# metagentools/VStrains

Measured on AMD Instinct MI355X. Metric: PE read pairs/sec through PE-link inference (GFA index + packed reads in HBM -> node_mat/short_mat), higher is better.
Workload: dtype u32

## Files before the change

vstrains_amd/csrc/vs_pe.hip:

```cpp
#include <stdio.h>
#include <stdlib.h>
#include <string.h>

#include <vector>

#include "vs_internal.h"
#include "vs_acc_tasks.h"
#include "vs_pe_pack.h"

#define TPB 256
#define LCAP 20u
__device__ __forceinline__ const uint32_t *vs_row_quad(const uint32_t *__restrict__ lists, const uint32_t *__restrict__ hi, uint64_t row, uint32_t q) {
    return q < LC / 4u ? lists + row * LC + 4u * q : hi + row * 4u;
}
#define EMPTY_NODE 0xFFFFFFFFu

struct PeParams {
    VsIndexDev idx;
    VsReadsDev rd;
    uint32_t *node_mat, *short_mat;
    unsigned long long *stats;
    uint32_t ept, pmax, words_cap, pool, pool_bits;
    uint64_t n_tiles;
    uint32_t *slow_list, *slow_count;
// ... 531 lines not shown
            __syncthreads();
            if (it < NI) {
                s_pcnt[it] = cnt;
                s_pa[it] = pa;
                s_pb[it] = pb;
            }
        } else
        for (uint32_t it = ltop; it < NI; it += TTPB) {
            uint32_t e = STD ? it / STD_PMAX : vs_fastdiv(it, P.magic_pmax), pi = it - e * pmax;
            uint32_t cnt = 0, pa = 0, pb = 0;
            const uint32_t est = e < ne ? s_state[e] : 0u;
            if ((est & 3u) == 1u) {
                uint32_t meta = s_meta[e];
                uint32_t rlen = meta & VS_LEN_MASK;
                uint32_t j = (est >> 8) + pi * s;
                if (j + w <= rlen) {
                    uint32_t sr;
                    const uint64_t key = vs_seed_key(s_words, e * wpe * 16u + j, w, &sr);
                    bool ok = true;
                    if ((meta >> 24) & VS_FLAG_INVALID) {
                        if (FAST) {
                            uint32_t lo, hi;
                            ok = vs_seed_limits(s_inv[e], j, w, rlen, &lo, &hi);
                        } else {
                            ok = !vs_seed_dirty(P.rd.mask, (uint64_t)s_gwoff[e] * 16u + j, w);
                        }
                    }
                    if (ok) cnt = vs_probe(P.idx, key, sr, &pa, &pb);
                }
            }
            s_pcnt[it] = cnt;
            s_pa[it] = pa;
            s_pb[it] = pb;
        }
        __syncthreads();
        {
            const uint32_t chunk = (NI + TTPB - 1u) / TTPB;
            const uint32_t b = ltop * chunk;
            uint32_t local = 0;
            for (uint32_t i = 0; i < chunk; i++)
                if (b + i < NI) local += s_pcnt[b + i];
            const uint32_t incl = vs_wave_scan_add(local);
            const uint32_t lane = ltop & 63u;
            if (lane == 63u) s_misc[ltop >> 6] = incl;
            __syncthreads();
            uint32_t off = incl - local;
            for (uint32_t wv = 0; wv < (ltop >> 6); wv++) off += s_misc[wv];
            for (uint32_t i = 0; i < chunk; i++)
                if (b + i < NI) {
                    off += s_pcnt[b + i];
                    s_pcnt[b + i] = off;
                }
        }
        __syncthreads();
        {
        const uint32_t total = s_pcnt[NI - 1u];
        for (uint32_t c0 = 0; c0 < total; c0 += KCHUNK) {
            for (uint32_t i = tid; i < KCHUNK; i += TTPB) s_owner[i] = 0;
            __syncthreads();
            for (uint32_t it = tid; it < NI; it += TTPB) {
                const uint32_t incl = s_pcnt[it], excl = s_pcnt[(int)it - 1];
                if (incl > excl) {
                    const uint32_t lo = excl > c0 ? excl : c0;
                    const uint32_t hi = incl < c0 + KCHUNK ? incl : c0 + KCHUNK;
                    if (lo < hi) s_owner[lo - c0] = it + 1u;
                }
            }
            __syncthreads();
            uint32_t own[KPPT];
            uint32_t run = 0;
#pragma unroll
            for (uint32_t k2 = 0; k2 < KPPT; k2++) {
                const uint32_t v = s_owner[tid * KPPT + k2];
                run = v > run ? v : run;
                own[k2] = run;
            }
            const uint32_t incl = vs_wave_scan_max(run);
            const uint32_t lane = tid & 63u;
            if (lane == 63u) s_misc[4u + (tid >> 6)] = incl;
            uint32_t carry = __shfl_up(incl, 1, 64);
            if (lane == 0u) carry = 0;
            __syncthreads();
            {
                const uint32_t wv = tid >> 6;
#pragma unroll
                for (uint32_t pw = 0; pw + 1u < TTPB / 64u; pw++) {
                    const uint32_t mw = s_misc[4u + pw];
                    if (wv > pw) carry = mw > carry ? mw : carry;
                }
            }
            bool live[KPPT];
            uint32_t p_e[KPPT], p_j[KPPT], p_node[KPPT], p_pos[KPPT], p_opp[KPPT];
            VsNodeMeta p_nm[KPPT];
#pragma unroll
            for (uint32_t k2 = 0; k2 < KPPT; k2++) {
                const uint32_t t = c0 + tid * KPPT + k2;
                live[k2] = t < total;
                const uint32_t it = live[k2] ? (own[k2] > carry ? own[k2] : carry) - 1u : 0u;
                const uint32_t excl = s_pcnt[(int)it - 1];
                const uint32_t cnt = s_pcnt[it] - excl;
                const uint32_t pa = s_pa[it], pb = s_pb[it];
                const uint32_t e = STD ? it / STD_PMAX : vs_fastdiv(it, P.magic_pmax), pi = it - e * pmax;
                p_e[k2] = e;
                uint32_t gap = s;
                {
                    const uint32_t est = s_state[e];
                    if (ADAPT) {
                        const uint32_t D = est >> 20, t = (est >> 16) & 15u;
                        p_j[k2] = ((est >> 8) & 0xFFu) + pi * s - (pi >= t ? D : 0u);
                        if (pi && pi == t) gap = s - D;
                    } else {
                        p_j[k2] = (est >> 8) + pi * s;
                    }
                }
                uint32_t node = pa, pos = pb & 0x7FFFFFFFu, opp = pb >> 31;
                p_nm[k2].woff = 0; p_nm[k2].len = 0;
                if (live[k2] && cnt != 1u) {
                    const VsPosting po = vs_posting_unpack(P.idx.postings[pa + (t - excl)]);
                    node = po.node; pos = po.pos; opp = po.strand ^ (pb >> 31);
                    p_nm[k2].woff = po.woff; p_nm[k2].len = po.len;
                } else if (live[k2]) {
                    if (P.shortcut && s <= w && pi) {
                        const uint32_t excl2 = s_pcnt[(int)it - 2];
                        if (excl - excl2 == 1u && s_pa[it - 1u] == node) {
                            const uint32_t pbp = s_pb[it - 1u];
                            const uint32_t want = opp ? pos + gap : pos - gap;
                            if ((pbp >> 31) == opp && (pbp & 0x7FFFFFFFu) == want && (opp || pos >= gap)) live[k2] = false;
                        }
                    }
                    if (live[k2]) p_nm[k2] = P.idx.meta[node];
                }
                p_node[k2] = node; p_pos[k2] = pos; p_opp[k2] = opp;
                if (ADAPT) p_j[k2] |= gap << 16;
            }
#pragma unroll
            for (uint32_t k2 = 0; k2 < KPPT; k2++) {
                if (!live[k2]) continue;
                const uint32_t e = p_e[k2], j = ADAPT ? p_j[k2] & 0xFFFFu : p_j[k2], node = p_node[k2], opp = p_opp[k2];
                const uint32_t gap = ADAPT ? p_j[k2] >> 16 : s;
                VsNodeMeta nm = p_nm[k2];
                const uint32_t meta = s_meta[e];
                const uint32_t rlen = meta & VS_LEN_MASK;
                const uint32_t *tw = P.idx.fwd_words;
                const uint32_t q = opp ? nm.len - p_pos[k2] - w : p_pos[k2];
                uint32_t a, qa, len;
                if (FAST) {
                    uint32_t lo = 0u, hi = rlen;
                    if ((meta >> 24) & VS_FLAG_INVALID) vs_seed_limits(s_inv[e], j, w, rlen, &lo, &hi);
                    uint32_t cl = gap < j - lo ? gap : j - lo;
                    cl = cl < q ? cl : q;
                    uint32_t rem = hi - j - wv;
                    const uint32_t dr = nm.len - q - wv;
                    rem = rem < dr ? rem : dr;
                    uint32_t left = 0u, ext = 0u;
                    const uint32_t tb = (nm.woff + (opp ? P.idx.rc_delta : 0u)) * 16u;
                    if (MODE == 2) vs_agree_long(s_words, e * wpe * 16u, tw, tb + q, cl, tb + q + wv, rem, j, wv, &left, &ext);
                    else vs_agree_fast<STD>(s_words, e * wpe * 16u, tw, tb + q, cl, tb + q + wv, rem, j, wv, &left, &ext);
                    len = left + wv + ext;
                    if (left >= gap || len < K) continue;
                    a = j - left;
                    qa = q - left;
                } else {
                    const uint32_t tb = (nm.woff + (opp ? P.idx.rc_delta : 0u)) * 16u;
                    const uint32_t *mk = ((meta >> 24) & VS_FLAG_INVALID) ? P.rd.mask : nullptr;
                    if (!vs_extend(s_words, e * wpe * 16u, rlen, tw, tb, nm.len, j, q, wv, s, K, mk, (uint64_t)s_gwoff[e] * 16u, &a, &qa, &len))
                        continue;
                }
                credit(e, node, nm.len, len - K + 1u, opp ? nm.len - qa - len : qa, a);
            }
            __syncthreads();
        }
        }
        __builtin_amdgcn_s_waitcnt(0x0F70);
        __syncthreads();
        uint32_t lt = tid;
        asm volatile("" : "+v"(lt));
        constexpr uint32_t SPT = STD ? C_POOL / TTPB : 1u;
        uint32_t r_key[SPT], r_at[SPT];
        auto judge = [&](uint32_t i, uint32_t key) -> uint32_t {
            const uint32_t e = key >> 25, node = key & 0x01FFFFFFu;
            const uint32_t rlen = s_meta[e] & VS_LEN_MASK;
            const uint32_t hj = s_hminj[i];
            const uint32_t nlen = FAST ? hj >> AB : P.idx.meta[node].len;
            const uint32_t minj = FAST ? hj & ((1u << AB) - 1u) : hj;
            if (FAST ? vs_accept32(s_hcnt[i], s_hminp[i], minj, nlen, rlen, K) : vs_accept(s_hcnt[i], s_hminp[i], minj, nlen, rlen, K))
                return atomicAdd(&s_ns[e], 1u);
            return 0xFFFFFFFFu;
        };
        if (STD) {
#pragma unroll
            for (uint32_t j = 0; j < SPT; j++) {
                const uint32_t i = lt + j * TTPB;
                r_key[j] = s_hkey[i];
                r_at[j] = r_key[j] != EMPTY_NODE ? judge(i, r_key[j]) : 0xFFFFFFFFu;
            }
        } else {
            for (uint32_t i = lt; i < pool; i += TTPB) {
                const uint32_t key = s_hkey[i];
                if (key != EMPTY_NODE) s_hcnt[i] = judge(i, key);
            }
        }
        __syncthreads();
        if (lt < 64u) {
            const uint32_t e0 = 2u * lt, e1 = e0 + 1u;
            const uint32_t st0 = e0 < ne ? s_state[e0] : 0u, st1 = e1 < ne ? s_state[e1] : 0u;
            const uint32_t n0 = (st0 & 3u) == 1u ? s_ns[e0] : 0u, n1 = (st1 & 3u) == 1u ? s_ns[e1] : 0u;
            bool over0 = n0 > LCAP, over1 = n1 > LCAP;
            const uint32_t q0 = over0 ? 0u : (n0 + 3u) >> 2, q1 = over1 ? 0u : (n1 + 3u) >> 2;
            const uint32_t incl = vs_wave_scan_add(q0 + q1);
            const uint32_t capq = (ept * LC - C_TRIM) >> 2;
            const uint32_t o0 = incl - q0 - q1, o1 = o0 + q0;
            over0 |= o0 + q0 > capq;
            over1 |= o1 + q1 > capq;
            if (e0 < ne) { s_pcnt[e0] = over0 || (st0 & 3u) != 1u ? 0xFFFFFFFFu : 4u * o0; if (over0) s_state[e0] = st0 | 2u; }
            if (e1 < ne) { s_pcnt[e1] = over1 || (st1 & 3u) != 1u ? 0xFFFFFFFFu : 4u * o1; if (over1) s_state[e1] = st1 | 2u; }
            if (lt == 63u) s_misc[8] = 4u * (incl < capq ? incl : capq);
        }
        __syncthreads();
        uint32_t *s_off = s_pcnt;
        if (STD) {
#pragma unroll
            for (uint32_t j = 0; j < SPT; j++)
                if (r_at[j] != 0xFFFFFFFFu) {
                    const uint32_t o = s_off[r_key[j] >> 25];
                    if (o != 0xFFFFFFFFu) s_list[o + r_at[j]] = r_key[j] & 0x01FFFFFFu;
                }
        } else {
            for (uint32_t i = lt; i < pool; i += TTPB) {
                const uint32_t key = s_hkey[i];
                if (key != EMPTY_NODE) {
                    const uint32_t at = s_hcnt[i], o = s_off[key >> 25];
                    if (at != 0xFFFFFFFFu && o != 0xFFFFFFFFu) s_list[o + at] = key & 0x01FFFFFFu;
                }
            }
        }
        __syncthreads();
        if (lt < npair) {
            uint32_t st = s_state[2 * lt] | s_state[2 * lt + 1];
            if ((st & 1u) && (st & 2u)) {
                uint32_t at = atomicAdd(P.slow_count, 1u);
                P.slow_list[at] = s_gend[2 * lt] >> 1;
                s_state[2 * lt] |= 2u;
                s_state[2 * lt + 1] |= 2u;
            }
        }
        __syncthreads();
        if (accumulate) {
            if (!P.out_rows) {
                uint32_t *ol = P.out_lists + (uint64_t)tile * ept * LC;
                const uint32_t total = s_misc[8];
                for (uint32_t i = lt; i < total; i += TTPB) ol[i] = s_list[i];
                for (uint32_t i = lt; i < ne; i += TTPB) {
                    const uint32_t n = (s_state[i] & 3u) == 1u ? s_ns[i] : 0u;
                    P.out_counts[(uint64_t)tile * ept + i] = n ? n | (s_off[i] >> 2) << 8 : 0u;
                }
            } else {
                uint32_t *ol = P.out_lists + (uint64_t)tile * ept * LC, *oh = P.out_lists_hi + (uint64_t)tile * ept * 4u;
                for (uint32_t i = lt; i < ne * (LCAP / 4u); i += TTPB) {
                    const uint32_t e = i / (LCAP / 4u), q4 = 4u * (i - e * (LCAP / 4u));
                    const uint32_t n = (s_state[e] & 3u) == 1u ? s_ns[e] : 0u;
                    if (q4 < n) {
                        const uint32_t *src = s_list + s_off[e] + q4;
                        *(VsQuad *)(q4 < LC ? ol + e * LC + q4 : oh + e * 4u) = VsQuad{src[0], src[1], src[2], src[3]};
                    }
                }
                for (uint32_t i = lt; i < ne; i += TTPB)
                    P.out_counts[(uint64_t)tile * ept + i] = (s_state[i] & 3u) == 1u ? s_ns[i] : 0u;
            }
        }
        if (want_dbg) {
            for (uint32_t i = tid; i < ne; i += TTPB) {
                if (s_state[i] & 2u) continue;
                uint32_t n = s_ns[i];
                const uint64_t ge = s_gend[i];
                P.dbg_counts[ge] = n;
                for (uint32_t k2 = 0; k2 < n && k2 < P.dbg_cap; k2++) P.dbg_lists[ge * P.dbg_cap + k2] = s_list[s_off[i] + k2];
            }
        }
    }
    __syncthreads();
    if (tid < 3 && P.stats && s_misc[12 + tid]) atomicAdd(&P.stats[tid], (unsigned long long)s_misc[12 + tid]);
}

#define ACC_LDS_BYTES ((2u * ACC_SLOTS + (ACC_TPB / 64) * (ACC_TASK_WORDS + ACC_BINS) + 4u) * 4u)
static_assert(ACC_LDS_BYTES <= 160u * 1024u, "k_pe_accumulate: one workgroup per CU");
template <uint32_t BITS>
struct CellTable {
    static constexpr uint32_t EMPTY = 0xFFFFFFFFu;
    __device__ static uint32_t key(uint32_t mat, uint32_t x, uint32_t y, uint32_t N) { return (mat * N + x) * N + y; }
    __device__ static uint32_t slot(uint32_t k) { return ((((k >> 4) * 0x9E3779B1u) >> (36u - BITS)) << 4) | (k & 15u); }
    __device__ static uint32_t next(uint32_t at) { return (at + 16u) & ((1u << BITS) - 1u); }
};
typedef CellTable<ACC_BITS> Acc32;

template <typename TB>
__device__ __forceinline__ bool vs_cell_claim(uint32_t *s_key, uint32_t *s_cnt, uint32_t *s_used, uint32_t key, uint32_t at, uint32_t wgt) {
    for (uint32_t pr = 0; pr < 8u; pr++) {
        uint32_t kx = s_key[at];
        if (kx == TB::EMPTY) {
            kx = atomicCAS(&s_key[at], TB::EMPTY, key);
            if (kx == TB::EMPTY) { atomicAdd(s_used, 1u); kx = key; }
        }
        if (kx == key) {
            atomicAdd(&s_cnt[at], wgt);
            return true;
        }
        at = TB::next(at);
    }
    return false;
}

template <typename TB>
__device__ __forceinline__ bool vs_cell_claim_seen(uint32_t *s_key, uint32_t *s_cnt, uint32_t *s_used, uint32_t key, uint32_t at, uint32_t wgt, uint32_t seen) {
    uint32_t kx = seen;
    for (uint32_t pr = 0; pr < 8u; pr++) {
        if (pr) kx = s_key[at];
        if (kx == TB::EMPTY) {
            kx = atomicCAS(&s_key[at], TB::EMPTY, key);
            if (kx == TB::EMPTY) { atomicAdd(s_used, 1u); kx = key; }
        }
        if (kx == key) {
            atomicAdd(&s_cnt[at], wgt);
            return true;
        }
        at = TB::next(at);
    }
    return false;
}

__device__ __forceinline__ void vs_wave_lds_sync() {
    __builtin_amdgcn_fence(__ATOMIC_RELEASE, "workgroup");
    __builtin_amdgcn_wave_barrier();
    __builtin_amdgcn_fence(__ATOMIC_ACQUIRE, "workgroup");
}

__global__ void __launch_bounds__(ACC_TPB)
k_pe_accumulate(const uint32_t *__restrict__ lists, const uint32_t *__restrict__ counts, uint64_t n_slots_pairs,
                uint32_t pairs_per_wg, uint32_t N, uint32_t use_table, uint32_t fill_limit, uint32_t task_cap,
                uint32_t *__restrict__ node_mat, uint32_t *__restrict__ short_mat, uint32_t *__restrict__ queue, uint32_t ept) {
    const uint32_t tid = threadIdx.x, lane = tid & 63u, wv = tid >> 6;
    uint32_t *s_key = vs_lds;
    uint32_t *s_cnt = vs_lds + ACC_SLOTS;
    uint32_t *s_bin = vs_lds + 2u * ACC_SLOTS + wv * (ACC_TASK_WORDS + ACC_BINS);
    uint16_t *s_task = (uint16_t *)(s_bin + ACC_BINS);
    uint32_t *s_misc = vs_lds + 2u * ACC_SLOTS + (ACC_TPB / 64) * (ACC_TASK_WORDS + ACC_BINS);
    uint32_t &s_used = s_misc[0], &s_lost = s_misc[1], &s_chunk = s_misc[2];
    const uint32_t NN = N * N;
    for (uint32_t i = tid; i < ACC_SLOTS; i += ACC_TPB) { s_key[i] = Acc32::EMPTY; s_cnt[i] = 0; }
    if (tid == 0) { s_used = 0; s_lost = 0; }
    __syncthreads();
    const uint32_t ppt = ept >> 1, region_q = (ept * LC) >> 2;
    auto write_out = [&]() {
        for (uint32_t i = tid; i < ACC_SLOTS; i += ACC_TPB) {
            const uint32_t key = s_key[i];
            if (key != Acc32::EMPTY) {
                atomicAdd(key >= NN ? short_mat + (key - NN) : node_mat + key, s_cnt[i]);
                s_key[i] = Acc32::EMPTY;
                s_cnt[i] = 0;
            }
        }
        if (tid == 0) { s_used = 0; s_lost = 0; }
        __syncthreads();
    };
    for (;;) {
    __syncthreads();
    if (tid == 0) s_chunk = atomicAdd(queue, 1u);
    __syncthreads();
    const uint64_t chunk = s_chunk;
    const uint64_t lo = chunk * pairs_per_wg;
    if (lo >= n_slots_pairs) break;
    const uint64_t hi = lo + pairs_per_wg < n_slots_pairs ? lo + pairs_per_wg : n_slots_pairs;
    for (uint64_t base = lo; base < hi; base += (ACC_TPB / 64u) * ACC_PPW) {
        const uint64_t wbase = base + wv * ACC_PPW;
        const uint32_t *wcounts = counts + 2u * wbase;
        const uint64_t tile0 = wbase / ppt;
        const uint32_t rem0 = (uint32_t)(wbase - tile0 * ppt);
        const uint32_t *wlists = lists + tile0 * ept * LC;
        uint32_t nl = 0, nr = 0, packed = 0;
        if (wbase + lane < hi) {
            const uint2 c = *(const uint2 *)(wcounts + 2u * lane);
            nl = c.x & 0xFFu; nr = c.y & 0xFFu;
            const uint32_t tq = (rem0 + lane) / ppt * region_q;
            packed = nl | nr << 5 | (tq + (c.x >> 8)) << 10 | (tq + (c.y >> 8)) << 21;
        }
        const uint32_t my_tasks = vs_acc_pair_tasks(nl, nr);
        for (uint32_t first = 0; first < ACC_PPW;) {
            const uint32_t incl = vs_wave_scan_add(lane >= first ? my_tasks : 0u);
            const uint32_t last = (uint32_t)__popcll(__ballot(vs_acc_batch_fits(incl, task_cap)));
            const uint32_t U = (uint32_t)__builtin_amdgcn_readlane((int)incl, (int)last - 1);
            const bool mine = lane >= first && lane < last;
            first = last;
            if (!U) continue;
            if (lane < ACC_BINS) s_bin[lane] = 0u;
            vs_wave_lds_sync();
            uint32_t o_n = 0, o_lm = 0, o_rm = 0, o_l[4], o_r[4];
            if (mine) {
                if (nl && nr) o_n = atomicAdd(&s_bin[nr], nl);
                if (nl & 1u) o_lm = atomicAdd(&s_bin[(nl + 1u) >> 1], 1u);
                if (nr & 1u) o_rm = atomicAdd(&s_bin[(nr + 1u) >> 1], 1u);
#pragma unroll
                for (uint32_t r = 0; r < 4u; r++) {
                    const VsAccClass cl = vs_acc_fold_class(nl, r), cr = vs_acc_fold_class(nr, r);
                    o_l[r] = cl.cnt ? atomicAdd(&s_bin[cl.turns], cl.cnt) : 0u;
                    o_r[r] = cr.cnt ? atomicAdd(&s_bin[cr.turns], cr.cnt) : 0u;
                }
            }
            vs_wave_lds_sync();
            {
                const uint32_t v = lane < ACC_BINS ? s_bin[ACC_BINS - 1u - lane] : 0u;
                const uint32_t before = vs_wave_scan_add(v) - v;
                if (lane < ACC_BINS) s_bin[ACC_BINS - 1u - lane] = before;
            }
            vs_wave_lds_sync();
            if (mine) {
                if (nl && nr) {
                    const uint32_t at = s_bin[nr] + o_n;
                    for (uint32_t a = 0; a < nl; a++) s_task[at + a] = vs_acc_task_entry(lane, VS_ACC_NODE, a);
                }
                if (nl & 1u) s_task[s_bin[(nl + 1u) >> 1] + o_lm] = vs_acc_task_entry(lane, VS_ACC_LEFT, nl >> 1);
                if (nr & 1u) s_task[s_bin[(nr + 1u) >> 1] + o_rm] = vs_acc_task_entry(lane, VS_ACC_RIGHT, nr >> 1);
                uint32_t nl2 = nl, nr2 = nr;
                asm volatile("" : "+v"(nl2), "+v"(nr2));
#pragma unroll
                for (uint32_t r = 0; r < 4u; r++) {
                    const VsAccClass cl = vs_acc_fold_class(nl2, r), cr = vs_acc_fold_class(nr2, r);
                    if (cl.cnt) {
                        const uint32_t at = s_bin[cl.turns] + o_l[r];
                        for (uint32_t i = 0; i < cl.cnt; i++) s_task[at + i] = vs_acc_task_entry(lane, VS_ACC_LEFT, cl.a0 + 4u * i);
                    }
                    if (cr.cnt) {
                        const uint32_t at = s_bin[cr.turns] + o_r[r];
                        for (uint32_t i = 0; i < cr.cnt; i++) s_task[at + i] = vs_acc_task_entry(lane, VS_ACC_RIGHT, cr.a0 + 4u * i);
                    }
                }
            }
            vs_wave_lds_sync();
            struct Task {
                uint32_t x, mat, off, p, p2, e, turns;
                VsQuad q;
            };
            auto decode = [&](uint32_t t0) {
                Task T;
                const uint32_t w = t0 + lane < U ? s_task[t0 + lane] : 0u;
                const uint32_t kind = vs_acc_entry_kind(w), a = vs_acc_entry_a(w);
                const uint32_t pk = __shfl(packed, (int)vs_acc_entry_pair(w), 64);
                const uint32_t ql = pk & 31u, qr = (pk >> 5) & 31u, rowl = ((pk >> 10) & 0x7FFu) << 2, rowr = (pk >> 21) << 2;
                const VsAccSegs s = w ? vs_acc_task_segs(kind, a, ql, qr) : VsAccSegs{0u, 0u, 0u};
                T.turns = vs_acc_turns(s);
                T.mat = kind != VS_ACC_NODE ? 1u : 0u;
                T.off = !w ? 0u : kind == VS_ACC_LEFT ? rowl : rowr;
                T.p = s.p1; T.p2 = s.p2; T.e = s.e;
                T.x = 0u;
                if (w && kind == VS_ACC_NODE) T.x = wlists[rowl + a];
                T.q = *(const VsQuad *)(wlists + T.off + T.p);
                return T;
            };
            Task nxt = decode(0u);
            for (uint32_t t0 = 0; t0 < U; t0 += 64u) {
                const Task c = nxt;
                if (t0 + 64u < U) nxt = decode(t0 + 64u);
                const uint32_t tmax = (uint32_t)__builtin_amdgcn_readlane((int)vs_wave_scan_max(c.turns), 63);
                const uint32_t mat = c.mat, e = c.e;
                const uint32_t *plist = wlists + c.off;
                uint32_t x = c.x, p = c.p, p2 = c.p2;
                bool fresh = true;
                VsQuad q = c.q;
                for (uint32_t t = 0; t < tmax; t += 4u) {
                    const uint32_t ys[4] = {q.x, q.y, q.z, q.w};
                    if (mat && fresh) x = ys[0];
                    const uint32_t pb = p;
                    p += 4u;
                    fresh = p >= e;
                    if (fresh) { p = p2; p2 = e; }
                    if (t + 4u < tmax) q = *(const VsQuad *)(plist + p);
                    const uint32_t left = tmax - t;
                    if (use_table) {
                        uint32_t key[4], seen[4], at[4];
#pragma unroll
                        for (uint32_t j = 0; j < 4u; j++) {
                            if (j >= left) break;
                            const uint32_t yv = ys[j];
                            const uint32_t cx = (mat && yv < x) ? yv : x, cy = (mat && yv < x) ? x : yv;
                            key[j] = Acc32::key(mat, cx, cy, N);
                            at[j] = Acc32::slot(key[j]);
                            seen[j] = s_key[at[j]];
                        }
#pragma unroll
                        for (uint32_t j = 0; j < 4u; j++) {
                            if (j >= left) break;
                            if (pb + j >= e) continue;
                            if (seen[j] == key[j]) {
                                atomicAdd(&s_cnt[at[j]], 1u);
                            } else if (!vs_cell_claim_seen<Acc32>(s_key, s_cnt, &s_used, key[j], at[j], 1u, seen[j])) {
                                atomicAdd(&s_lost, 1u);
                                atomicAdd(key[j] >= NN ? short_mat + (key[j] - NN) : node_mat + key[j], 1u);
                            }
                        }
                    } else {
#pragma unroll
                        for (uint32_t j = 0; j < 4u; j++) {
                            if (pb + j >= e) continue;
                            const uint32_t yv = ys[j];
                            const uint32_t cx = (mat && yv < x) ? yv : x, cy = (mat && yv < x) ? x : yv;
                            atomicAdd((mat ? short_mat : node_mat) + (uint64_t)cx * N + cy, 1u);
                        }
                    }
                }
            }
        }
        __syncthreads();
        const bool spill = s_used > fill_limit || s_lost > 4096u;
        __syncthreads();
        if (spill) write_out();
    }
    }
    __syncthreads();
    write_out();
}

__global__ void __launch_bounds__(256) k_mark_tiles(const uint32_t *__restrict__ lists, const uint32_t *__restrict__ counts,
                                                   uint64_t n_slots_pairs, uint8_t *__restrict__ map, uint32_t T, uint32_t ept) {
    const uint64_t p = (uint64_t)blockIdx.x * blockDim.x + threadIdx.x;
    if (p >= n_slots_pairs) return;
    const uint32_t cl = counts[2u * p], cr = counts[2u * p + 1u], nl = cl & 0xFFu, nr = cr & 0xFFu;
    if (!nl && !nr) return;
    const uint32_t *region = lists + 2u * p / ept * ept * LC, *rl = region + 4u * (cl >> 8), *rr = region + 4u * (cr >> 8);
    uint8_t *smap = map + (uint64_t)T * T;
    uint32_t tl[8], tr[8], kl = 0, kr = 0;
    bool over = false;
    auto put = [&](uint32_t (&tt)[8], uint32_t &k, uint32_t t) {
        bool seen = false;
#pragma unroll
        for (uint32_t j = 0; j < 8u; j++) seen |= j < k && tt[j] == t;
        if (seen) return;
        if (k >= 8u) { over = true; return; }
#pragma unroll
        for (uint32_t j = 0; j < 8u; j++)
            if (j == k) tt[j] = t;
        k++;
    };
#pragma unroll
    for (uint32_t j = 0; j < 8u; j++) { tl[j] = 0u; tr[j] = 0u; }
#pragma unroll
    for (uint32_t q = 0; q < LCAP / 4u; q++) {
        if (4u * q < nl) {
            const VsQuad v = *(const VsQuad *)(rl + 4u * q);
            const uint32_t e[4] = {v.x, v.y, v.z, v.w};
#pragma unroll
            for (uint32_t i = 0; i < 4u; i++)
                if (4u * q + i < nl) put(tl, kl, e[i] >> 6);
        }
        if (4u * q < nr) {
            const VsQuad v = *(const VsQuad *)(rr + 4u * q);
            const uint32_t e[4] = {v.x, v.y, v.z, v.w};
#pragma unroll
            for (uint32_t i = 0; i < 4u; i++)
                if (4u * q + i < nr) put(tr, kr, e[i] >> 6);
        }
    }
    if (over) {
        for (uint32_t i = 0; i < nl; i++)
            for (uint32_t j = 0; j < nr; j++) vs_mark_tile(map, T, 0u, rl[i], rr[j]);
        for (uint32_t side = 0; side < 2u; side++) {
            const uint32_t *row = side ? rr : rl;
            const uint32_t n = side ? nr : nl;
            for (uint32_t i = 0; i < n; i++)
                for (uint32_t j = 0; j < n; j++) {
                    const uint32_t x = row[i], y = row[j];
                    if (x <= y) vs_mark_tile(map, T, 1u, x, y);
                }
        }
        return;
    }
#pragma unroll
    for (uint32_t a = 0; a < 8u; a++)
#pragma unroll
        for (uint32_t b = 0; b < 8u; b++)
            if (a < kl && b < kr) {
                const uint64_t t = (uint64_t)tl[a] * T + tr[b];
                if (!map[t]) map[t] = 1;
            }
#pragma unroll
    for (uint32_t a = 0; a < 8u; a++)
#pragma unroll
        for (uint32_t b = 0; b < 8u; b++) {
            if (a < kl && b < kl && tl[a] <= tl[b]) {
                const uint64_t t = (uint64_t)tl[a] * T + tl[b];
                if (!smap[t]) smap[t] = 1;
            }
            if (a < kr && b < kr && tr[a] <= tr[b]) {
                const uint64_t t = (uint64_t)tr[a] * T + tr[b];
                if (!smap[t]) smap[t] = 1;
            }
        }
}

__global__ void __launch_bounds__(64) k_zero_tiles(uint32_t *__restrict__ node_mat, uint32_t *__restrict__ short_mat, uint32_t N, uint32_t T,
                                                  uint8_t *__restrict__ map, uint64_t n_tiles) {
    const uint64_t t0 = (uint64_t)blockIdx.x * 64u;
    const uint64_t mine = t0 + threadIdx.x;
    const bool marked = mine < n_tiles && map[mine] != 0;
    unsigned long long todo = __ballot(marked);
    if (marked) map[mine] = 0;
    while (todo) {
        const uint32_t k = (uint32_t)__ffsll((long long)todo) - 1u;
        todo &= todo - 1ull;
        const uint64_t t = t0 + k;
        const uint32_t mat = (uint32_t)(t / ((uint64_t)T * T));
        const uint64_t r = t - (uint64_t)mat * T * T;
        const uint32_t x0 = (uint32_t)(r / T) << 6, y = (((uint32_t)(r % T)) << 6) + threadIdx.x;
        uint32_t *m = mat ? short_mat : node_mat;
        if (y < N)
            for (uint32_t x = x0; x < x0 + 64u && x < N; x++) m[(uint64_t)x * N + y] = 0u;
    }
}

#define ROWS_CHUNK 16384u
#define ROWS_CHUNK1 8192u
#define ROWS_TPB 1024u
#define ROWS_CAP 4096u
static inline size_t rows_lds_bytes(uint32_t n_keys) { return sizeof(uint32_t) * (((size_t)n_keys + 2u) / 2u + ROWS_CAP + ROWS_CAP / 2u + 4u); }

#define LTAB_PROBES 16u
__device__ __forceinline__ void vs_load_list(const uint32_t *__restrict__ row, const uint32_t *__restrict__ hi, uint32_t n, uint32_t (&v)[LCAP]) {
    const VsQuad z{0, 0, 0, 0};
    const VsQuad a = *(const VsQuad *)row, b = n > 4u ? *(const VsQuad *)(row + 4) : z, c = n > 8u ? *(const VsQuad *)(row + 8) : z;
    const VsQuad d = n > 12u ? *(const VsQuad *)(row + 12) : z, f = n > 16u ? *(const VsQuad *)hi : z;
    const uint32_t w[LCAP] = {a.x, a.y, a.z, a.w, b.x, b.y, b.z, b.w, c.x, c.y, c.z, c.w, d.x, d.y, d.z, d.w, f.x, f.y, f.z, f.w};
#pragma unroll
    for (uint32_t i = 0; i < LCAP; i++) v[i] = i < n ? w[i] : 0xFFFFFFFFu;
}
__device__ __forceinline__ bool vs_same_list(const uint32_t (&mine)[LCAP], const uint32_t (&other)[LCAP], uint32_t n) {
    bool same = true;
    if (n <= LC) {
#pragma unroll
        for (uint32_t k2 = 0; k2 < LC; k2++) {
            bool found = false;
#pragma unroll
            for (uint32_t i = 0; i < LC; i++) found |= mine[i] == other[k2];
            same &= found || k2 >= n;
        }
        return same;
    }
#pragma unroll
    for (uint32_t k2 = 0; k2 < LCAP; k2++) {
        bool found = false;
#pragma unroll
        for (uint32_t i = 0; i < LCAP; i++) found |= mine[i] == other[k2];
        same &= found || k2 >= n;
    }
    return same;
}

__global__ void __launch_bounds__(256)
k_list_owners(const uint32_t *__restrict__ lists, const uint32_t *__restrict__ lists_hi, const uint32_t *__restrict__ counts, uint64_t n_ends, uint32_t *__restrict__ mult,
              uint32_t *__restrict__ gown, unsigned long long *__restrict__ ltab, uint32_t *__restrict__ lmult, uint32_t ltab_bits) {
    const uint64_t e64 = (uint64_t)blockIdx.x * blockDim.x + threadIdx.x;
    if (e64 >= n_ends) return;
    const uint32_t e = (uint32_t)e64, n = counts[e];
    uint32_t m = n ? 1u : 0u, own = e;
    if (n && ltab) {
        uint32_t mine[LCAP];
        vs_load_list(lists + e64 * LC, lists_hi + e64 * 4u, n, mine);
        unsigned long long f2 = n;
#pragma unroll
        for (uint32_t i = 0; i < LCAP; i++)
            if (i < n) {
                unsigned long long g = (mine[i] + 1ull) * 0x9E3779B97F4A7C15ull;
                g ^= g >> 29;
                f2 += g * 0xBF58476D1CE4E5B9ull;
            }
        const uint32_t tag = ((uint32_t)(f2 >> 32) & ~31u) | (n - 1u);
        const unsigned long long word = ((unsigned long long)tag << 32) | (e + 1u);
        uint32_t h = (uint32_t)((f2 * 0xD6E8FEB86659FD93ull) >> (64u - ltab_bits));
        for (uint32_t pr = 0; pr < LTAB_PROBES; pr++) {
            unsigned long long cur = ltab[h];
            if (cur == 0ull) {
                cur = atomicCAS(&ltab[h], 0ull, word);
                if (cur == 0ull) {
                    atomicAdd(&lmult[h], 1u);
                    m = 0u;
                    break;
                }
            }
            if ((uint32_t)(cur >> 32) == tag) {
                uint32_t other[LCAP];
                vs_load_list(lists + (uint64_t)((uint32_t)cur - 1u) * LC, lists_hi + (uint64_t)((uint32_t)cur - 1u) * 4u, n, other);
                if (vs_same_list(mine, other, n)) {
                    atomicAdd(&lmult[h], 1u);
                    m = 0u;
                    own = (uint32_t)cur - 1u;
                    break;
                }
            }
            h = (h + 1u) & ((1u << ltab_bits) - 1u);
        }
    }
    mult[e] = m;
    gown[e] = own;
}

__global__ void __launch_bounds__(256)
k_owners_mult(const unsigned long long *__restrict__ ltab, const uint32_t *__restrict__ lmult, uint64_t n_slots, uint32_t *__restrict__ mult) {
    const uint64_t h = (uint64_t)blockIdx.x * blockDim.x + threadIdx.x;
    if (h >= n_slots) return;
    const unsigned long long w = ltab[h];
    if (w != 0ull) mult[(uint32_t)w - 1u] = lmult[h];
}

#define COLLECT_TPB 256u
__global__ void __launch_bounds__(COLLECT_TPB)
k_owners_collect(const uint32_t *__restrict__ mult, uint64_t n_ends, uint64_t per_wg, uint32_t *__restrict__ owners, uint32_t *__restrict__ n_owners) {
    __shared__ uint32_t s_wave[COLLECT_TPB / 64u], s_base;
    const uint32_t tid = threadIdx.x, lane = tid & 63u, wv = tid >> 6;
    const uint64_t lo = (uint64_t)blockIdx.x * per_wg, hi = lo + per_wg < n_ends ? lo + per_wg : n_ends;
    uint32_t mine = 0;
    for (uint64_t e = lo + tid; e < hi; e += COLLECT_TPB) mine += mult[e] != 0u ? 1u : 0u;
#pragma unroll
    for (int d = 32; d; d >>= 1) mine += __shfl_xor(mine, d, 64);
    if (lane == 0) s_wave[wv] = mine;
    __syncthreads();
    if (tid == 0) {
        uint32_t tot = 0;
        for (uint32_t i = 0; i < COLLECT_TPB / 64u; i++) tot += s_wave[i];
        s_base = tot ? atomicAdd(n_owners, tot) : 0u;
        s_wave[0] = 0u;
    }
    __syncthreads();
    for (uint64_t e0 = lo; e0 < hi; e0 += COLLECT_TPB) {
        const uint64_t e = e0 + tid;
        const bool own = e < hi && mult[e] != 0u;
        const unsigned long long live = __ballot(own);
        uint32_t wbase = 0;
        if (lane == 0 && live) wbase = atomicAdd(&s_wave[0], (uint32_t)__popcll(live));
        wbase = __shfl(wbase, 0, 64);
        if (own) owners[s_base + wbase + (uint32_t)__popcll(live & ((1ull << lane) - 1ull))] = (uint32_t)e;
    }
}

template <int MODE>
__device__ __forceinline__ uint32_t vs_rows_item(const uint32_t *__restrict__ counts, const uint32_t *__restrict__ owners, uint64_t i, uint64_t &row) {
    if (MODE == 0) {
        const uint2 c = *(const uint2 *)(counts + 2u * i);
        row = 2u * i;
        return c.y ? c.x : 0u;
    }
    row = owners[i];
    return counts[row];
}

template <int MODE>
__device__ __forceinline__ void vs_rows_histogram(uint32_t *h32, const uint32_t *__restrict__ lists, const uint32_t *__restrict__ lists_hi, const uint32_t *__restrict__ counts,
                                                  const uint32_t *__restrict__ owners, uint64_t lo, uint64_t hi, uint32_t key_lo, uint32_t n_keys) {
    for (uint64_t i = lo * 4u + threadIdx.x; i < hi * 4u; i += ROWS_TPB) {
        uint64_t row;
        const uint32_t q0 = (uint32_t)i & 3u, n = vs_rows_item<MODE>(counts, owners, i >> 2, row);
        for (uint32_t q = q0; 4u * q < n; q += 4u) {
            const VsQuad v = *(const VsQuad *)vs_row_quad(lists, lists_hi, row, q);
            const uint32_t e[4] = {v.x, v.y, v.z, v.w};
#pragma unroll
            for (uint32_t j = 0; j < 4u; j++) {
                const uint32_t x = e[j] - key_lo;
                if (4u * q + j < n && x < n_keys) atomicAdd(&h32[x >> 1], 1u << ((x & 1u) * 16u));
            }
        }
    }
}

template <int MODE>
__global__ void __launch_bounds__(ROWS_TPB)
k_rows_count(const uint32_t *__restrict__ lists, const uint32_t *__restrict__ lists_hi, const uint32_t *__restrict__ counts, const uint32_t *__restrict__ owners, uint64_t n_items,
             const uint32_t *__restrict__ n_owners, uint32_t key_lo, uint32_t n_keys, uint32_t *__restrict__ row_count) {
    uint32_t *h32 = vs_lds;
    const uint32_t words = (n_keys + 1u) >> 1, tid = threadIdx.x;
    if (MODE) n_items = *n_owners;
    const uint64_t per = MODE ? ROWS_CHUNK1 : ROWS_CHUNK;
    const uint64_t lo = (uint64_t)blockIdx.x * per, hi = lo + per < n_items ? lo + per : n_items;
    if (lo >= n_items) return;
    for (uint32_t i = tid; i < words; i += ROWS_TPB) h32[i] = 0u;
    __syncthreads();
    vs_rows_histogram<MODE>(h32, lists, lists_hi, counts, owners, lo, hi, key_lo, n_keys);
    __syncthreads();
    for (uint32_t i = tid; i < words; i += ROWS_TPB) {
        const uint32_t v = h32[i];
        if (v & 0xFFFFu) atomicAdd(&row_count[key_lo + 2u * i], v & 0xFFFFu);
        if (v >> 16) atomicAdd(&row_count[key_lo + 2u * i + 1u], v >> 16);
    }
}

template <int MODE>
__global__ void __launch_bounds__(ROWS_TPB)
k_rows_fill(const uint32_t *__restrict__ lists, const uint32_t *__restrict__ lists_hi, const uint32_t *__restrict__ counts, const uint32_t *__restrict__ owners, uint64_t n_items,
            const uint32_t *__restrict__ n_owners, const uint32_t *__restrict__ gown, uint32_t key_lo, uint32_t n_keys,
            const uint32_t *__restrict__ row_ptr, uint32_t *__restrict__ row_cursor, uint32_t *__restrict__ entries) {
    uint32_t *h32 = vs_lds;
    const uint32_t words = (n_keys + 1u) >> 1, tid = threadIdx.x;
    if (MODE) n_items = *n_owners;
    if ((uint64_t)blockIdx.x * (MODE ? ROWS_CHUNK1 : ROWS_CHUNK) >= n_items) return;
    uint32_t *s_base = h32 + words;
    uint32_t *s_fill = s_base + ROWS_CAP;
    uint32_t &s_nc = s_fill[ROWS_CAP / 2u];
    for (uint32_t i = tid; i < words; i += ROWS_TPB) h32[i] = 0u;
    for (uint32_t i = tid; i < ROWS_CAP / 2u; i += ROWS_TPB) s_fill[i] = 0u;
    if (tid == 0) s_nc = 0u;
    __syncthreads();
    const uint64_t per = MODE ? ROWS_CHUNK1 : ROWS_CHUNK;
    const uint64_t lo = (uint64_t)blockIdx.x * per, hi = lo + per < n_items ? lo + per : n_items;
    vs_rows_histogram<MODE>(h32, lists, lists_hi, counts, owners, lo, hi, key_lo, n_keys);
    __syncthreads();
    for (uint32_t i = tid; i < words; i += ROWS_TPB) {
        const uint32_t v = h32[i];
        if (!v) continue;
// ... 1326 lines not shown
```

vstrains_amd/csrc/vs_pe_plan.h:

```cpp
#ifndef VS_PE_PLAN_H
#define VS_PE_PLAN_H
#include <stddef.h>
#include <stdint.h>
#include <stdio.h>

#include <initializer_list>

#include "../../include/vstrains_hip.h"

#if defined(__HIPCC__)
#define VS_PLAN_FN __host__ __device__ inline
#else
#define VS_PLAN_FN inline
#endif

struct VsTuning {
    uint32_t ept = 0;
    uint32_t grid_per_cu = 128;
    int acc_fill_pct = -1;
    uint32_t acc_tasks = 0;
    int shortcut = -1;
    int adapt_grid = -1;
    int acc_rows = -1;
    int ltab_bits = -1;
    uint32_t rows_keys = 0, rows_sub = 0;
    uint32_t rows_per_strip = 0;
    bool no_sort = false, locus_global = false, no_fast = false, no_std = false, no_agg = false;
    bool no_mid = false;
    int locus_stage = -1;
};

VS_PLAN_FN uint32_t vs_seed_phase(uint32_t len, uint32_t w, uint32_t s) {
    return len < w ? 0u : ((len - w) % s + s) / 2u;
}
VS_PLAN_FN uint32_t vs_seed_probes(uint32_t len, uint32_t w, uint32_t s) {
    if (len < w) return 0u;
    return (len - w + 1u) / s;
}
#define VS_SEED_VERIFIED(w) ((w) <= 31u ? (w) : 0u)

#define LC 16u
#define PPT 2u
#define TTPB 256
#define PPT_LONG 1u
#define CHUNK (TTPB * PPT)
#define ACC_TPB 1024
#define ACC_BITS 14
#define ACC_SLOTS (1u << ACC_BITS)
#define ACC_PPW 64u
#define ACC_TASK_WORDS 480u
#define ACC_TASK_CAP (2u * ACC_TASK_WORDS)
#define ACC_TASK_MIN 40u
#define ACC_BINS 24u
#define ROWS_KEYS 65536u
#define ROWS_SUB ((1u << 26) - 1024u)
#define RS_BITS 13
#define RS_SLOTS (1u << RS_BITS)
#define LOCUS_LDS_KEYS 36864u
#define LOCUS_LDS_MAX_PASSES 4u
#define LOCUS_WGS 256u
#define LOCUS_STAGE_WAVES 16u
#define LOCUS_STAGE_PAIRS 64u
#define LOCUS_STAGE_QUADS 5u
#define LOCUS_STAGE_SLACK 16u
#define LOCUS_STAGE_MAX (LOCUS_STAGE_QUADS * 4u * LOCUS_STAGE_PAIRS - LOCUS_STAGE_SLACK)
#define LOCUS_STAGE_MIN_PAIRS 48u
#define LOCUS_LDS_WORDS 40960u
#define SLOW_WORDS_PER_NODE 6u
#define LDS_BUDGET_BYTES (64u * 1024u)
#define NI_CAP 4096u

VS_PLAN_FN bool vs_locus_in_batch(bool exists, uint32_t w_first, uint32_t w_pair_end, uint32_t cap) {
    return exists && w_pair_end - w_first <= cap;
}
struct LocusBatch {
    uint32_t n;
    uint32_t staged;
};
VS_PLAN_FN LocusBatch vs_locus_batch(const uint32_t *woff, uint64_t p0, uint64_t hi, uint32_t cap) {
    LocusBatch b = {0u, 1u};
    if (p0 >= hi) return b;
    const uint32_t w_first = woff[2u * p0];
    while (b.n < LOCUS_STAGE_PAIRS && vs_locus_in_batch(p0 + b.n < hi, w_first, p0 + b.n < hi ? woff[2u * (p0 + b.n) + 2u] : 0u, cap)) b.n++;
    if (!b.n) { b.n = 1u; b.staged = 0u; }
    return b;
}
struct LocusSpan {
    uint32_t first, quads;
};
VS_PLAN_FN LocusSpan vs_locus_span(uint32_t w_first, uint32_t w_end) {
    LocusSpan sp;
    sp.first = w_first & ~3u;
    sp.quads = (w_end + 4u - sp.first + 3u) / 4u;
    return sp;
}
VS_PLAN_FN uint32_t vs_locus_buf_words(uint32_t cap) { return ((cap + 3u) & ~3u) + LOCUS_STAGE_SLACK; }

struct TileLayout {
    uint32_t woff, gend, meta, inv, words, pcnt, pa, pb, hkey, hcnt, hminp, hminj, ns, state, list, owner, misc, total;
};
VS_PLAN_FN TileLayout tile_layout(uint32_t ept, uint32_t pmax, uint32_t words_cap, uint32_t pool, uint32_t list_trim = 0u) {
    TileLayout t;
    uint32_t o = 0;
    const uint32_t NI = ept * pmax;
    t.woff = o;  o += 2u * ((ept + 2u) & ~1u);
    t.gend = o;  o += 2u * ept;
    t.meta = o;  o += 2u * ept;
    t.inv = o;   o += ept;
    t.words = o; o += 2u * (words_cap + 8u);
    t.pcnt = o;  o += NI + 1u;
    t.pa = o;    o += NI;
    t.pb = o;    o += NI;
    t.hkey = o;  o += pool;
    t.hcnt = o;  o += pool;
    t.hminp = o; o += pool;
    t.hminj = o; o += pool;
    t.ns = o;    o += ept;
    t.state = o; o += ept;
    t.list = o;
    t.owner = o; o += (ept * LC - list_trim > CHUNK ? ept * LC - list_trim : CHUNK);
    t.misc = o;  o += 16u;
    t.total = o;
    return t;
}

#define STD_EPT (TTPB / 4u)
#define STD_POOL_BITS 10u
#define STD_K 56u
#define STD_W 31u
#define STD_S 26u
#define STD2_EPT 60u
#define STD2_POOL_BITS 10u
#define STD2_K 128u
#define STD2_W 63u
#define STD2_S 66u
struct StdShape {
    uint32_t mode, sw, sp;
};
constexpr StdShape VS_STD_SHAPES[] = {{1u, 10u, 4u}, {1u, 8u, 3u}, {1u, 7u, 2u}, {1u, 7u, 3u}, {2u, 16u, 2u}};
struct StdTable {
    uint32_t pool, trim;
};
VS_PLAN_FN constexpr StdTable vs_std_table(int mode, bool std_shape, bool ad) {
    return std_shape && !ad ? StdTable{768u, mode == 2 ? 192u : 64u} : StdTable{1u << (mode == 2 ? STD2_POOL_BITS : STD_POOL_BITS), 0u};
}

inline uint32_t slow_grid_for(uint32_t n_nodes) {
    const uint64_t per_wg = sizeof(uint32_t) * (uint64_t)SLOW_WORDS_PER_NODE * (n_nodes ? n_nodes : 1u);
    uint64_t g = (4ull << 30) / per_wg;
    return (uint32_t)(g < 64u ? 64u : g > 2048u ? 2048u : g);
}

inline uint32_t pool_for(uint32_t ept, uint32_t *bits) {
    uint32_t b = 6;
    while ((1u << b) < 16u * ept) b++;
    *bits = b;
    return 1u << b;
}

inline size_t lds_bytes(uint32_t ept, uint32_t pmax, uint32_t words_cap) {
    uint32_t bits;
    uint32_t pool = pool_for(ept, &bits);
    return (size_t)tile_layout(ept, pmax, words_cap, pool).total * sizeof(uint32_t);
}

struct PePlanIn {
    uint32_t n_nodes = 0, K = 0, w = 0, s = 0;
    uint64_t n_seed_pos = 0, n_distinct = 0;
    uint32_t max_node_len = 0, n_cu = 0;
    uint64_t n_ends = 0;
    uint32_t max_len = 0;
    bool has_mask = false, has_inv4 = false;
    bool count = false, tile_map = false;
    VsTuning tune;
};

struct PePlan {
    int status;
    char msg[128];
    uint32_t ept, pmax, wpe, pool, pool_bits, words_cap, magic_pmax, magic_wpe;
    uint64_t lds_bytes;
    uint32_t mode, sw, sp, ad;
    uint64_t n_tiles, grid, list_ends, list_words;
    uint32_t tiles_per_wg, shortcut, mid_fast;
    uint32_t use_sort, lds_sort, locus_chunk, locus_per_pass;
    uint64_t locus_keys, locus_hist_words;
    uint32_t locus_stage_words;
    uint64_t locus_lds_bytes;
    uint32_t use_rows, use_table, mark_tiles;
    uint32_t acc_grid, acc_per_wg, acc_fill, acc_task_cap;
    uint64_t rows_sub_pairs;
    uint32_t rows_ltab_bits, rows_keys, rows_fill, rows_per_strip;
    uint32_t slow_grid;
    uint64_t dense_bytes;
};

inline PePlan vs_pe_plan(const PePlanIn &in) {
    PePlan p = {};
    const VsTuning &tn = in.tune;
    const uint64_t n_pairs = in.n_ends / 2;
    if (n_pairs == 0) return p;
    const uint32_t maxlen = in.max_len, N = in.n_nodes;
    if (N > 0x01FFFFFEu) {
        p.status = VS_E_RANGE;
        snprintf(p.msg, sizeof p.msg, "more than 2^25-2 nodes");
        return p;
    }
    const uint32_t wpe = maxlen ? (maxlen + 15u) / 16u : 1u;
    uint32_t pmax = vs_seed_probes(maxlen, in.w, in.s);
    if (!pmax) pmax = 1u;
    uint32_t ept = tn.ept ? tn.ept : STD_EPT;
    if (ept < 2 || ept > TTPB / 2u) ept = STD_EPT;
    while (ept > 2 && (ept * pmax > NI_CAP || lds_bytes(ept, pmax, ept * wpe) > LDS_BUDGET_BYTES)) ept -= 2;
    if (!tn.ept) {
        for (size_t fit : {(size_t)32000, (size_t)40000}) {
            uint32_t e2 = ept;
            while (e2 > STD_EPT / 2u && lds_bytes(e2, pmax, e2 * wpe) > fit) e2 -= 2;
            if (lds_bytes(e2, pmax, e2 * wpe) <= fit) { ept = e2; break; }
        }
    }
    size_t lds = lds_bytes(ept, pmax, ept * wpe);
    if (lds > 160u * 1024u) {
        p.status = VS_E_RANGE;
        snprintf(p.msg, sizeof p.msg, "reads of %u bases with k+1=%u need %zu B of LDS per pair (limit 160 KiB)", maxlen, in.K, lds);
        return p;
    }
    p.ept = ept;
    p.pmax = pmax;
    p.wpe = wpe;
    p.words_cap = ept * wpe;
    p.pool = pool_for(ept, &p.pool_bits);
    p.magic_pmax = pmax > 1u ? (uint32_t)(0x100000000ull / pmax) + 1u : 0u;
    p.magic_wpe = wpe > 1u ? (uint32_t)(0x100000000ull / wpe) + 1u : 0u;
    p.slow_grid = slow_grid_for(N);
    p.dense_bytes = sizeof(uint32_t) * (uint64_t)SLOW_WORDS_PER_NODE * (N ? N : 1) * p.slow_grid;

    p.use_sort = !tn.no_sort && n_pairs >= 4096 && n_pairs < 0xFFFFFFF0ull;
    if (p.use_sort) {
        const uint64_t nk = (uint64_t)N + 2u;
        const bool fits_lds = nk <= LOCUS_LDS_MAX_PASSES * LOCUS_LDS_KEYS;
        p.locus_keys = nk;
        p.locus_hist_words = fits_lds ? nk * LOCUS_WGS : nk;
        p.lds_sort = fits_lds && !tn.locus_global;
        if (p.lds_sort) {
            p.locus_chunk = (uint32_t)((n_pairs + LOCUS_WGS - 1) / LOCUS_WGS);
            p.locus_per_pass = (uint32_t)(nk < LOCUS_LDS_KEYS ? nk : LOCUS_LDS_KEYS);
            p.locus_lds_bytes = sizeof(uint32_t) * (uint64_t)p.locus_per_pass;
            if (nk < LOCUS_LDS_KEYS && tn.locus_stage != 0) {
                const uint32_t hist = ((uint32_t)nk + 3u) & ~3u;
                uint32_t room = ((LOCUS_LDS_WORDS - hist) / (2u * LOCUS_STAGE_WAVES) - LOCUS_STAGE_SLACK) & ~3u;
                if (room > LOCUS_STAGE_MAX) room = LOCUS_STAGE_MAX;
                uint32_t cap = room / (2u * wpe) >= LOCUS_STAGE_MIN_PAIRS ? room : 0u;
                if (tn.locus_stage > 0) cap = (uint32_t)tn.locus_stage < room ? (uint32_t)tn.locus_stage : room;
                if (cap) {
                    p.locus_stage_words = cap;
                    p.locus_lds_bytes = sizeof(uint32_t) * (uint64_t)(hist + 2u * LOCUS_STAGE_WAVES * vs_locus_buf_words(cap));
                }
            }
        }
    }

    p.use_table = tn.no_agg ? 0u : 1u;
    const bool fits32 = 2ull * N * N < 0xFFFFFFFFull;
    bool use_rows = tn.acc_rows >= 0 ? tn.acc_rows != 0 : !fits32;
    if (N == 0 || !p.use_table) use_rows = false;
    if (!use_rows && !fits32) p.use_table = 0u;
    p.use_rows = use_rows;
    p.n_tiles = (n_pairs + ept / 2 - 1) / (ept / 2);
    p.list_ends = p.n_tiles * ept;
    p.list_words = p.list_ends * (use_rows ? LC + 4u : LC) + 16u;

    p.shortcut = in.n_distinct && in.n_seed_pos < 2 * in.n_distinct ? 1u : 0u;
    if (tn.shortcut >= 0) p.shortcut = (uint32_t)tn.shortcut;
    if (VS_SEED_VERIFIED(in.w) == 0u) p.shortcut = 0u;

    const bool straight = (!in.has_mask || in.has_inv4) && in.max_node_len < (1u << 23) && !tn.no_fast;
    const bool fast = straight && in.s <= 32u && maxlen <= 128u + in.w + 32u;
    p.mid_fast = fast && VS_SEED_VERIFIED(in.w) ? 1u : 0u;
    uint32_t long_reach = 0;
    for (uint32_t len = in.K; len <= maxlen; len++) {
        const uint32_t behind = len - vs_seed_phase(len, in.w, in.s) - VS_SEED_VERIFIED(in.w);
        long_reach = behind > long_reach ? behind : long_reach;
    }
    const bool fast_long = !fast && straight && in.s <= 128u && long_reach <= 256u && maxlen < 512u;
    p.mode = fast ? 1u : fast_long ? 2u : 0u;
    const bool shape1 = p.mode == 1u && ept == STD_EPT && p.pool_bits == STD_POOL_BITS && maxlen <= 159u && in.K == STD_K && in.w == STD_W && in.s == STD_S;
    const bool shape2 = p.mode == 2u && ept == STD2_EPT && p.pool_bits == STD2_POOL_BITS && in.K == STD2_K && in.w == STD2_W && in.s == STD2_S;
    if (in.count && !tn.no_std && (shape1 || shape2))
        for (const StdShape &sh : VS_STD_SHAPES)
            if (sh.mode == p.mode && sh.sw == wpe && sh.sp == pmax) { p.sw = wpe; p.sp = pmax; }
    if (p.sw) {
        p.ad = tn.adapt_grid >= 0 ? tn.adapt_grid != 0 : in.n_distinct && in.n_seed_pos >= 6u * in.n_distinct;
        const StdTable tab = vs_std_table((int)p.mode, true, p.ad);
        lds = (size_t)tile_layout(ept, pmax, ept * wpe, tab.pool, tab.trim).total * sizeof(uint32_t);
    }
    p.lds_bytes = lds;
    const uint64_t max_grid = (uint64_t)in.n_cu * tn.grid_per_cu;
    p.grid = p.n_tiles < max_grid ? p.n_tiles : max_grid;
    p.tiles_per_wg = (uint32_t)((p.n_tiles + p.grid - 1) / p.grid);
    p.grid = (p.n_tiles + p.tiles_per_wg - 1) / p.tiles_per_wg;
    if (!in.count) return p;

    const uint64_t slots_pairs = p.list_ends / 2;
    if (!use_rows) {
        p.mark_tiles = in.tile_map;
        p.acc_grid = in.n_cu * 32u;
        p.acc_per_wg = (uint32_t)((slots_pairs + p.acc_grid - 1) / p.acc_grid);
        p.acc_per_wg = (p.acc_per_wg + ACC_TPB - 1) / ACC_TPB * ACC_TPB;
        p.acc_grid = (uint32_t)((slots_pairs + p.acc_per_wg - 1) / p.acc_per_wg);
        if (p.acc_grid > in.n_cu * 2u) p.acc_grid = in.n_cu * 2u;
        p.acc_fill = ACC_SLOTS / 16u;
        if (tn.acc_fill_pct >= 0) p.acc_fill = (uint32_t)((uint64_t)ACC_SLOTS * (uint32_t)tn.acc_fill_pct / 100u);
        p.acc_task_cap = tn.acc_tasks >= ACC_TASK_MIN && tn.acc_tasks < ACC_TASK_CAP ? tn.acc_tasks : ACC_TASK_CAP;
        return p;
    }
    const uint64_t sub_max = tn.rows_sub ? (uint64_t)tn.rows_sub : (uint64_t)ROWS_SUB;
    p.rows_sub_pairs = slots_pairs < sub_max ? slots_pairs : sub_max;
    p.rows_ltab_bits = 10;
    while ((1ull << p.rows_ltab_bits) < 2u * p.rows_sub_pairs && p.rows_ltab_bits < 31u) p.rows_ltab_bits++;
    if (tn.ltab_bits >= 0) p.rows_ltab_bits = (uint32_t)tn.ltab_bits;
    const uint32_t keys_max = tn.rows_keys ? tn.rows_keys : ROWS_KEYS;
    p.rows_keys = N < keys_max ? N : keys_max;
    p.rows_fill = RS_SLOTS / 2u;
    if (tn.acc_fill_pct >= 0) p.rows_fill = (uint32_t)((uint64_t)RS_SLOTS * (uint32_t)tn.acc_fill_pct / 100u);
    if (p.rows_fill > RS_SLOTS - 1024u) p.rows_fill = RS_SLOTS - 1024u;
    p.rows_per_strip = tn.rows_per_strip ? tn.rows_per_strip : 2u;
    return p;
}

#endif
```

Measured before the change: 1.459 billion.

## Defer LDS hash-table misses to a per-wave queue drained in batches

In the accumulate kernel, lanes whose first-probe key does not match no longer run the CAS probe loop inline. The keys are compacted with ballot/mbcnt into a 64-entry per-wave LDS queue carved from the task buffer, and the queue is drained in bulk when it fills or at the end of each batch. This is meant to cut wave divergence from the serialized claim loop in the hot path. In exchange the task buffer cap shrinks to make room for the queue, and extra wave syncs and drain passes are added.

```diff
diff --git a/vstrains_amd/csrc/vs_pe.hip b/vstrains_amd/csrc/vs_pe.hip
--- a/vstrains_amd/csrc/vs_pe.hip
+++ b/vstrains_amd/csrc/vs_pe.hip
@@ -857,25 +857,7 @@
             if (kx == TB::EMPTY) { atomicAdd(s_used, 1u); kx = key; }
         }
         if (kx == key) {
-            atomicAdd(&s_cnt[at], wgt);
-            return true;
-        }
-        at = TB::next(at);
-    }
-    return false;
-}
-
-template <typename TB>
-__device__ __forceinline__ bool vs_cell_claim_seen(uint32_t *s_key, uint32_t *s_cnt, uint32_t *s_used, uint32_t key, uint32_t at, uint32_t wgt, uint32_t seen) {
-    uint32_t kx = seen;
-    for (uint32_t pr = 0; pr < 8u; pr++) {
-        if (pr) kx = s_key[at];
-        if (kx == TB::EMPTY) {
-            kx = atomicCAS(&s_key[at], TB::EMPTY, key);
-            if (kx == TB::EMPTY) { atomicAdd(s_used, 1u); kx = key; }
-        }
-        if (kx == key) {
-            atomicAdd(&s_cnt[at], wgt);
+            __hip_atomic_fetch_add(&s_cnt[at], wgt, __ATOMIC_RELAXED, __HIP_MEMORY_SCOPE_WORKGROUP);
             return true;
         }
         at = TB::next(at);
@@ -898,6 +880,7 @@
     uint32_t *s_cnt = vs_lds + ACC_SLOTS;
     uint32_t *s_bin = vs_lds + 2u * ACC_SLOTS + wv * (ACC_TASK_WORDS + ACC_BINS);
     uint16_t *s_task = (uint16_t *)(s_bin + ACC_BINS);
+    uint32_t *s_q = s_bin + ACC_BINS + (ACC_TASK_WORDS - ACC_QUEUE);
     uint32_t *s_misc = vs_lds + 2u * ACC_SLOTS + (ACC_TPB / 64) * (ACC_TASK_WORDS + ACC_BINS);
     uint32_t &s_used = s_misc[0], &s_lost = s_misc[1], &s_chunk = s_misc[2];
     const uint32_t NN = N * N;
@@ -916,6 +899,19 @@
         }
         if (tid == 0) { s_used = 0; s_lost = 0; }
         __syncthreads();
+    };
+    uint32_t qn = 0;
+    auto drain = [&]() {
+        vs_wave_lds_sync();
+        if (lane < qn) {
+            const uint32_t key = s_q[lane];
+            if (!vs_cell_claim<Acc32>(s_key, s_cnt, &s_used, key, Acc32::slot(key), 1u)) {
+                atomicAdd(&s_lost, 1u);
+                atomicAdd(key >= NN ? short_mat + (key - NN) : node_mat + key, 1u);
+            }
+        }
+        vs_wave_lds_sync();
+        qn = 0;
     };
     for (;;) {
     __syncthreads();
@@ -1043,12 +1039,16 @@
 #pragma unroll
                         for (uint32_t j = 0; j < 4u; j++) {
                             if (j >= left) break;
-                            if (pb + j >= e) continue;
-                            if (seen[j] == key[j]) {
-                                atomicAdd(&s_cnt[at[j]], 1u);
-                            } else if (!vs_cell_claim_seen<Acc32>(s_key, s_cnt, &s_used, key[j], at[j], 1u, seen[j])) {
-                                atomicAdd(&s_lost, 1u);
-                                atomicAdd(key[j] >= NN ? short_mat + (key[j] - NN) : node_mat + key[j], 1u);
+                            const bool on = pb + j < e;
+                            if (on && seen[j] == key[j]) atomicAdd(&s_cnt[at[j]], 1u);
+                            const bool miss = on && seen[j] != key[j];
+                            const uint64_t mm = __ballot(miss);
+                            if (mm) {
+                                const uint32_t n_miss = (uint32_t)__popcll(mm);
+                                if (qn + n_miss > ACC_QUEUE) drain();
+                                const uint32_t before = __builtin_amdgcn_mbcnt_hi((uint32_t)(mm >> 32), __builtin_amdgcn_mbcnt_lo((uint32_t)mm, 0u));
+                                if (miss) s_q[qn + before] = key[j];
+                                qn += n_miss;
                             }
                         }
                     } else {
@@ -1063,6 +1063,7 @@
                 }
             }
         }
+        if (qn) drain();
         __syncthreads();
         const bool spill = s_used > fill_limit || s_lost > 4096u;
         __syncthreads();
diff --git a/vstrains_amd/csrc/vs_pe_plan.h b/vstrains_amd/csrc/vs_pe_plan.h
--- a/vstrains_amd/csrc/vs_pe_plan.h
+++ b/vstrains_amd/csrc/vs_pe_plan.h
@@ -51,6 +51,8 @@
 #define ACC_TASK_WORDS 480u
 #define ACC_TASK_CAP (2u * ACC_TASK_WORDS)
 #define ACC_TASK_MIN 40u
+#define ACC_QUEUE 64u
+#define ACC_TASK_PLAN_CAP (ACC_TASK_CAP - 2u * ACC_QUEUE)
 #define ACC_BINS 24u
 #define ROWS_KEYS 65536u
 #define ROWS_SUB ((1u << 26) - 1024u)
@@ -311,7 +313,7 @@
         if (p.acc_grid > in.n_cu * 2u) p.acc_grid = in.n_cu * 2u;
         p.acc_fill = ACC_SLOTS / 16u;
         if (tn.acc_fill_pct >= 0) p.acc_fill = (uint32_t)((uint64_t)ACC_SLOTS * (uint32_t)tn.acc_fill_pct / 100u);
-        p.acc_task_cap = tn.acc_tasks >= ACC_TASK_MIN && tn.acc_tasks < ACC_TASK_CAP ? tn.acc_tasks : ACC_TASK_CAP;
+        p.acc_task_cap = tn.acc_tasks >= ACC_TASK_MIN && tn.acc_tasks < ACC_TASK_PLAN_CAP ? tn.acc_tasks : ACC_TASK_PLAN_CAP;
         return p;
     }
     const uint64_t sub_max = tn.rows_sub ? (uint64_t)tn.rows_sub : (uint64_t)ROWS_SUB;
```

After: 1.504 billion, median of 6. 3.1% higher.
